# tusen-ai/MV2D

Measured on AMD Instinct MI355X. Metric: multi-view samples/sec (6-cam frames) through the MV2D RoI-head hot path, higher is better.
Workload: dtype f16x3: every operand an fp16 hi + lo pair, three MFMAs per product, fp32 accumulation (fp32-class, index-exact route; the lo halves of the key / value rows are STORED as e4m3 bytes); 1 GPU; cfg2_s: MV2D-S head, 6 views 1408x512; global_batch=384, streams_per_gpu=4, samples_per_launch=16, pe_sine_branch=folded into a per-(weights, geometry) table, FLOPs not counted, parallelism=dp1, hipgraph=True

## Files before the change

include/mv2d_hip.h:

```cpp
#ifndef MV2D_HIP_H
#define MV2D_HIP_H
#ifdef __cplusplus
extern "C" {
#endif

const char* mv2d_last_error(void);
int mv2d_abi_version(void);
int mv2d_key16_format(void);
int mv2d_f32_to_key16(const float* x, void* hi, void* lo, long long n, void* stream);
int mv2d_device_arch(char* buf, int buflen);
int mv2d_spin(int usec, void* stream);


int mv2d_gemm_bf16(const void* A, const void* A2, int n_split, int a_mode, const void* W, const float* bias, int M, int N,
                   int K, int lda, const int* m_dev, int act, const float* mul, int ldmul, const float* add, int ldadd,
                   void* C, int c_bf16, int ldc, long long c_blk_stride, int c_blk_cols, void* C2, const float* add2,
                   int ldc2, int ldadd2, void* stream);
int mv2d_gemm_bf16_ex(const void* A, const void* A2, int n_split, int a_mode, const void* W, const float* bias, int M, int N, int K, int lda,
                      const int* m_dev, int act, const float* mul, int ldmul, const float* add, int ldadd, void* C, int c_bf16, int ldc,
                      long long c_blk_stride, int c_blk_cols, void* C2, const float* add2, int ldc2, int ldadd2, int c_split3, const int* add_idx , int add_period,
                      int k_splits , long long c_split_stride, void* stream);
int mv2d_split3_rows(const float* a, const float* b, void* out, int M, int cols, const int* m_dev, void* stream);

int mv2d_gemm_f32(const float* A, const float* A2, int n_split, const float* W, const float* bias, int M, int N, int K,
// ... 109 lines not shown
int mv2d_split_rows_key16(const float* a, const float* b, void* hi, void* lo, int M, int cols, const int* m_dev, void* stream);

int mv2d_heads_fused_x3(const float* outs, const void* const* cls_w, const void* const* reg_w, const float* ref, float* cls, float* reg,
                        int M, int L, float eps, const float* pc_range, float dt, const float* dt_rows, void* stream);
int mv2d_heads_fused_x3_nc(const float* outs, const void* const* cls_w, const void* const* reg_w, const float* ref, float* cls, float* reg,
                           int M, int L, int num_classes, float eps, const float* pc_range, float dt, const float* dt_rows, void* stream);
int mv2d_heads_cls_x3_nc(const float* outs, const void* const* cls_w, float* cls, int M, int L, int num_classes, float eps, void* stream);
int mv2d_reg_layer_x3(const float* outs, const void* const* w, const float* ref, float* reg, int M, int L, int n_groups, const int* group_dims,
                      const float* pc_range, float dt, const float* dt_rows, void* stream);

int mv2d_heads_depth_x3(const float* outs, const void* const* cls_w, const void* const* reg_w, const float* ref, float* cls, float* reg,
                        int M, int L, int n_fcs, int num_classes, float eps, const float* pc_range, float dt, const float* dt_rows, void* stream);
int mv2d_heads_cls_depth_x3(const float* outs, const void* const* cls_w, float* cls, int M, int L, int n_fcs, int num_classes, float eps,
                            void* stream);
int mv2d_reg_layer_depth_x3(const float* outs, const void* const* w, const float* ref, float* reg, int M, int L, int n_fcs, int n_groups,
                            const int* group_dims, const float* pc_range, float dt, const float* dt_rows, void* stream);

int mv2d_ffn_pack_weights(const float* W1, const float* W2, float* W1p, float* W2p, int hidden, void* stream);
int mv2d_ffn_fused(const float* X, const float* W1, const float* b1, const float* W2, float* slabs, int M, int hidden, void* stream);

int mv2d_ffn_fused_x3(const float* X, const void* W1hi, const void* W1lo, const float* b1, const void* W2hi, const void* W2lo,
                      float* slabs, int M, int hidden, int slices_per_block, void* stream);

int mv2d_split_bf16x2(const float* x, void* hi, void* lo, long long n, void* stream);
int mv2d_q16_format(void);
int mv2d_split_q16x2(const float* x, void* hi, void* lo, long long n, void* stream);


int mv2d_row_ln(const float* parts, int n_parts, long long part_stride, const float* bias, const float* residual,
                const float* ln_w, const float* ln_b, int relu, float* out, const float* addvec, float* out_plus,
                const float* ln2_w, const float* ln2_b, float* out2, int M, float eps, int rows_per_group, void* stream);

int mv2d_finalize_reg(float* reg, const float* ref, int L, int R, const float* pc_range, float dt, void* stream);

int mv2d_avgpool49(const float* x, float* out, int ld_out, int R, void* stream);

int mv2d_f32_to_bf16(const float* x, void* y, long long n, void* stream);

int mv2d_nchw_to_nhwc(const float* x, float* y, int V, int C, int HW, void* stream);
int mv2d_nchw_to_nhwc_masked(const float* x, float* y, const unsigned char* mask, int V, int C, int HW, void* stream);
int mv2d_nchw_to_nhwc_fmt(const void* x, void* y, int V, int C, int HW, int map_fmt, void* stream);
int mv2d_nchw_to_nhwc_masked_fmt(const void* x, void* y, const unsigned char* mask, int V, int C, int HW, int map_fmt, void* stream);

int mv2d_nchw_to_nhwc_bf16(const float* x, void* y, int V, int C, int HW, void* stream);
int mv2d_map_conv3x3(const void* in, const void* Wp, const float* bias, float* out, int V, int h, int w, void* stream);



int mv2d_self_attn_fwd(const float* qkv, float* ctx, int R, const int* grp_start, int n_samples, void* stream);

int mv2d_self_attn_x3_fwd(const float* qkv, float* ctx, int R, const int* grp_start, int n_samples, int max_grp_rows, int dn_pad,
                          int dn_single, void* stream);

int mv2d_self_attn_dn_fwd(const float* qkv, float* ctx, int R, int dn_pad, int dn_single, void* stream);

int mv2d_sparse_xattn_fwd(const float* q, const void* K, const void* V, const int* row_ptr, const int* col_idx, float* ctx,
                          float* dbg_logits, long long dbg_stride, int R, int empty_nan, void* stream);

int mv2d_xattn_qmap(const float* q, const void* WA_hi, const void* WA_lo, void* Qt, int R, void* stream);
int mv2d_xattn_tile_fwd(const void* Qt, const void* Xk, const void* Xv, const void* Xk_lo, const void* Xv_lo, const int* row_ptr,
                        const int* col_idx, float* z, float* dbg_logits, long long dbg_stride, int R, int empty_nan, int waves, void* stream);
int mv2d_xattn_tile_fwd_ordered(const void* Qt, const void* Xk, const void* Xv, const void* Xk_lo, const void* Xv_lo, const int* row_ptr,
                                const int* col_idx, float* z, float* dbg_logits, long long dbg_stride, int R, int empty_nan, int waves,
                                const int* order, int lo_fmt, void* stream);
int mv2d_xattn_fused_fwd(const float* q, const void* WA_hi, const void* WA_lo, const void* WB_hi, const void* WB_lo, const float* bv, const void* Xk,
                         const void* Xv, const void* Xk_lo, const void* Xv_lo, const int* row_ptr, const int* col_idx, float* ctx, int R, int empty_nan,
                         const int* order, int lo_fmt, void* stream);
int mv2d_xattn_group_max(int R, int n_samples);
int mv2d_xattn_group_tables(const int* row_ptr, const int* col_idx, const int* order, const int* grp_start, int n_samples, int R, int ng_max, int* g_slot,
                            int* g_cnt, int* g_ptr, int* g_len, int* ucol, unsigned char* umask, int ucap, int* u_total, int* flags, void* stream);
int mv2d_xattn_group_fwd(const float* q, const void* WA_hi, const void* WA_lo, const void* WB_hi, const void* WB_lo, const float* bv, const void* Xk,
                         const void* Xv, const void* Xk_lo, const void* Xv_lo, const int* row_ptr, const int* order, const int* g_slot, const int* g_cnt,
                         const int* g_ptr, const int* g_len, const int* ucol, const unsigned char* umask, float* ctx, int ng_max, int empty_nan,
                         void* stream);
int mv2d_xattn_ctxmap(const float* z, const void* WB_hi, const void* WB_lo, const float* bv, const int* row_ptr, float* ctx, int R,
                      int empty_nan, void* stream);

int mv2d_xattn_query_order(const int* row_ptr, const int* col_idx, const int* grp_start, int n_samples, int R, int* perm, int* flags, int stride,
                           void* stream);
int mv2d_attn_out_qmap_x3(const float* ctx, const float* resid, const void* Wo_hi, const void* Wo_lo, const float* bo, const float* ln_w,
                          const float* ln_b, float* x_out, const float* qpos, const void* Wq_hi, const void* Wq_lo, const float* bq,
                          float qscale, const void* WA_hi, const void* WA_lo, void* Qt, int M, float eps, void* stream);
int mv2d_attn_out_zmap_x3(const float* z, const void* WB_hi, const void* WB_lo, const float* bv, const int* row_ptr, int empty_nan,
                          const float* resid, const void* Wo_hi, const void* Wo_lo, const float* bo, const float* ln_w, const float* ln_b,
                          float* x_out, int M, float eps, void* stream);

int mv2d_sparse_xattn_bwd(const float* q, const void* K, const void* V, const int* row_ptr, const int* col_idx, const float* ctx,
                          const float* dctx, const int* key_ptr, const int* pair_idx, const int* pair_row, float* pair_ws,
                          float* dq, float* dK, float* dV, int R, int S, void* stream);
int mv2d_sparse_xattn_fwd_drop(const float* q, const void* K, const void* V, const int* row_ptr, const int* col_idx, float* ctx, float* dbg_logits,
                               long long dbg_stride, int R, int empty_nan, float p_drop, unsigned int seed, void* stream);
int mv2d_sparse_xattn_bwd_drop(const float* q, const void* K, const void* V, const int* row_ptr, const int* col_idx, const float* ctx,
                               const float* dctx, const int* key_ptr, const int* pair_idx, const int* pair_row, float* pair_ws, float* dq, float* dK,
                               float* dV, int R, int S, float p_drop, unsigned int seed, void* stream);
int mv2d_sparse_xattn_bwd_ex(const float* q, const void* K, const void* V, const int* row_ptr, const int* col_idx, const float* ctx, const float* dctx,
                             const int* key_ptr, const int* pair_idx, const int* pair_row, float* pair_ws, float* dq, float* dK, float* dV, int R,
                             int S, float p_drop, unsigned int seed, int long_rows, float dq_scale, void* stream);


int mv2d_box_params(const float* rois, const double* viewK, const double* viewE, double* K_roi, float* intr, int ld_intr,
                    float* minv, int R, float roi_size, float intr_scale, float min_size, void* stream);

int mv2d_refpoint_posemb(const float* center_pred, int ld_cp, const float* minv, const float* dim_t, float* xyz, float* ref,
                         float* posemb, int R, const float* pc_range, void* stream);

int mv2d_lidar2img_inverse(const double* K_roi, const double* E, float* minv, int R, void* stream);
// ... 174 lines not shown
```

mv2d_amd/_lib.py:

```python
import ctypes as C
import os

HERE = os.path.dirname(os.path.abspath(__file__))
LIB_PATH = os.path.join(HERE, 'lib', 'libmv2d_hip.so')


class Mv2dHipError(RuntimeError):
    pass


P, I, LL, F, D = C.c_void_p, C.c_int, C.c_longlong, C.c_float, C.c_double
ABI_VERSION = 6

class TdDims(C.Structure):
    _fields_ = [('T', I), ('S', I), ('L', I), ('F', I), ('sa_nnz', I), ('ca_nnz', I), ('p_sa_attn', F), ('p_sa_out', F), ('p_ca_attn', F),
                ('p_ca_out', F), ('p_ffn_act', F), ('p_ffn_out', F), ('seed', C.c_uint), ('eps', F), ('pad', I), ('nk', I)]


class ThDims(C.Structure):
    _fields_ = [('T', I), ('L', I), ('NC', I), ('eps', F)]


SIGNATURES = {
    'mv2d_last_error': (C.c_char_p, []),
# ... 12 lines not shown
    'mv2d_pe_fused_x3_ng': (I, [P, P, P, P, I] + [P] * 7 + [I] + [P] * 5 + [I, I, P, I, I, P]),
    'mv2d_pe_gate_x3': (I, [P, P, P, P, I] + [P] * 7 + [I] + [P] * 5 + [I, I, P]),
    'mv2d_pe_gate_rows_x3': (I, [P, P, P, P, I] + [P] * 7 + [I] + [P] * 5 + [I, P, I, P, I, I, P]),
    'mv2d_pe_fused_x3_k_sel': (I, [P, P, P, P, I] + [P] * 13 + [I] + [P] * 5 + [I, P, I, I, P, I, I, P]),
    'mv2d_pe_fused_x3b': (I, [P, P, P, P, I] + [P] * 13 + [I] + [P] * 5 + [I, I, P, P]),
    'mv2d_key16_format': (I, []),
    'mv2d_f32_to_key16': (I, [P, P, P, LL, P]),
    'mv2d_split_rows_key16': (I, [P, P, P, P, I, I, P, P]),
    'mv2d_qg_conv_pool': (I, [P, P, P, P, I, I, P]),
    'mv2d_qg_conv_pool_x3': (I, [P, P, P, P, P, P, I, I, P]),
    'mv2d_qg_conv_pool_s': (I, [P, P, P, P, I, I, I, P]),
    'mv2d_qg_conv_pool_x3_s': (I, [P, P, P, P, P, P, I, I, I, P]),
    'mv2d_qg_conv_cells': (I, [P, P, P, P, P, P, I, I, P]),
    'mv2d_qg_conv_cells_x3': (I, [P, P, P, P, P, P, P, P, I, I, P]),
    'mv2d_avgpool_cells': (I, [P, P, P, I, I, I, P]),
    'mv2d_pack_wfrag_bf16': (I, [P, P, I, I, P]),
    'mv2d_gemm_f32': (I, [P, P, I, P, P, I, I, I, I, I, I, I, F, F, P, I, I, LL, I, LL, LL, LL, LL, P]),
    'mv2d_attn_out_fused': (I, [P, P, P, P, P, P, P, P, P, P, F, P, I, F, P]),
    'mv2d_sa_block_fused_x3': (I, [P, P, P, P, P, P, P, P, P, P, P, P, F, P, I, F, P]),
    'mv2d_query_embed_fused_x3': (I, [P] * 17 + [I, P]),
    'mv2d_qg_tail_x3': (I, [P, P, I] + [P] * 25 + [I, P]),
    'mv2d_ffn_out_fused_x3': (I, [P, I, LL, P, P, P, P, P, P, P, P, P, P, P, P, P, P, I, F, P]),
    'mv2d_attn_out_fused_x3': (I, [P, P, P, P, P, P, P, P, P, P, P, P, F, P, I, F, P]),
    'mv2d_pack_wfrag_f32': (I, [P, P, I, I, I, P]),
    'mv2d_heads_fused': (I, [P, P, P, P, P, P, I, I, F, P, F, P, P]),
    'mv2d_linear_x3': (I, [P, P, I, I, P, P, P, P, I, I, I, I, I, F, I, LL, LL, LL, LL, P]),
    'mv2d_linear_x3_ex': (I, [P, P, I, I, P, P, P, P, I, I, I, I, I, F, I, LL, LL, LL, LL, P, I, P, P, I, P]),
    'mv2d_heads_fused_x3': (I, [P, P, P, P, P, P, I, I, F, P, F, P, P]),
    'mv2d_heads_fused_x3_nc': (I, [P, P, P, P, P, P, I, I, I, F, P, F, P, P]),
    'mv2d_heads_cls_x3_nc': (I, [P, P, P, I, I, I, F, P]),
    'mv2d_reg_layer_x3': (I, [P, P, P, P, I, I, I, P, P, F, P, P]),
    'mv2d_heads_depth_x3': (I, [P, P, P, P, P, P, I, I, I, I, F, P, F, P, P]),
    'mv2d_heads_cls_depth_x3': (I, [P, P, P, I, I, I, I, F, P]),
    'mv2d_reg_layer_depth_x3': (I, [P, P, P, P, I, I, I, I, P, P, F, P, P]),
    'mv2d_ffn_fused': (I, [P, P, P, P, P, I, I, P]),
    'mv2d_ffn_pack_weights': (I, [P, P, P, P, I, P]),
    'mv2d_ffn_fused_x3': (I, [P, P, P, P, P, P, P, I, I, I, P]),
    'mv2d_split_bf16x2': (I, [P, P, P, LL, P]),
    'mv2d_split_q16x2': (I, [P, P, P, LL, P]),
    'mv2d_q16_format': (I, []),
    'mv2d_row_ln': (I, [P, I, LL, P, P, P, P, I, P, P, P, P, P, P, I, F, I, P]),
    'mv2d_finalize_reg': (I, [P, P, I, I, P, F, P]),
    'mv2d_avgpool49': (I, [P, P, I, I, P]),
    'mv2d_f32_to_bf16': (I, [P, P, LL, P]),
    'mv2d_nchw_to_nhwc': (I, [P, P, I, I, I, P]),
    'mv2d_nchw_to_nhwc_masked': (I, [P, P, P, I, I, I, P]),
    'mv2d_nchw_to_nhwc_fmt': (I, [P, P, I, I, I, I, P]),
    'mv2d_nchw_to_nhwc_masked_fmt': (I, [P, P, P, I, I, I, I, P]),
    'mv2d_nchw_to_nhwc_bf16': (I, [P, P, I, I, I, P]),
    'mv2d_map_conv3x3': (I, [P, P, P, P, I, I, I, P]),
    'mv2d_self_attn_fwd': (I, [P, P, I, P, I, P]),
    'mv2d_self_attn_dn_fwd': (I, [P, P, I, I, I, P]),
    'mv2d_self_attn_x3_fwd': (I, [P, P, I, P, I, I, I, I, P]),
    'mv2d_dn_queries': (I, [P, P, P, I, I, F, F, F, I, P, F, P, P, P, P]),
    'mv2d_sparse_xattn_fwd': (I, [P, P, P, P, P, P, P, LL, I, I, P]),
    'mv2d_sparse_xattn_bwd': (I, [P] * 14 + [I, I, P]),
    'mv2d_sparse_xattn_fwd_drop': (I, [P, P, P, P, P, P, P, LL, I, I, F, C.c_uint, P]),
    'mv2d_sparse_xattn_bwd_drop': (I, [P] * 14 + [I, I, F, C.c_uint, P]),
    'mv2d_sparse_xattn_bwd_ex': (I, [P] * 14 + [I, I, F, C.c_uint, I, F, P]),
    'mv2d_dgrad_relu_f32x3': (I, [P, P, P, F, P, I, I, I, P]),
    'mv2d_xattn_qmap': (I, [P, P, P, P, I, P]),
    'mv2d_attn_out_qmap_x3': (I, [P] * 12 + [F, P, P, P, I, F, P]),
    'mv2d_attn_out_zmap_x3': (I, [P, P, P, P, P, I, P, P, P, P, P, P, P, I, F, P]),
    'mv2d_xattn_tile_fwd': (I, [P, P, P, P, P, P, P, P, P, LL, I, I, I, P]),
    'mv2d_xattn_tile_fwd_ordered': (I, [P, P, P, P, P, P, P, P, P, LL, I, I, I, P, I, P]),
    'mv2d_xattn_fused_fwd': (I, [P, P, P, P, P, P, P, P, P, P, P, P, P, I, I, P, I, P]),
    'mv2d_xattn_group_max': (I, [I, I]),
    'mv2d_xattn_group_tables': (I, [P, P, P, P, I, I, I, P, P, P, P, P, P, I, P, P, P]),
    'mv2d_xattn_group_fwd': (I, [P] * 19 + [I, I, P]),
    'mv2d_xattn_query_order': (I, [P, P, P, I, I, P, P, I, P]),
    'mv2d_xattn_ctxmap': (I, [P, P, P, P, P, P, I, I, P]),
    'mv2d_box_params': (I, [P, P, P, P, P, I, P, I, F, F, F, P]),
    'mv2d_refpoint_posemb': (I, [P, I, P, P, P, P, P, I, P, P]),
    'mv2d_lidar2img_inverse': (I, [P, P, P, I, P]),
    'mv2d_posemb3d': (I, [P, P, P, I, P]),
    'mv2d_roi_align': (I, [P, P, P, P, P, P, P, I, I, I, I, F, I, P, I, P]),
    'mv2d_roi_align_ex': (I, [P, P, P, P, P, P, P, I, I, I, I, F, I, P, I, P, P, P, P, P, P]),
    'mv2d_roi_align_s': (I, [P, P, P, P, P, P, P, I, I, I, I, F, I, P, I, P, P, P, P, P, I, P]),
    'mv2d_roi_align_fmt': (I, [P, P, P, P, P, P, P, I, I, I, I, F, I, P, I, P, P, P, P, P, I, I, P]),
    'mv2d_box_correlation': (I, [P, P, P, P, P, P, I, I, I, I, I, I, I, F, F, F, I, P]),
    'mv2d_csr_workspace_bytes': (LL, [I, I, I, I]),
    'mv2d_mask_compact': (I, [P, P, P, P, P, P, P, P, P, P, P, P, P, I, I, I, I, I, I, F, F, I, P]),
    'mv2d_roi_positions': (I, [P, P, P, P, P, P, P, I, I, I, I, F, F, P]),
    'mv2d_csr_from_corr': (I, [P, P, P, P, I, I, I, P]),
    'mv2d_csr_from_corr_s': (I, [P, P, P, P, I, I, I, I, P]),
    'mv2d_roi_positions_csr': (I, [P, P, P, P, P, P, P, I, I, I, I, F, F, P, P, P, P, I, I, P, I, P, P, P]),
    'mv2d_roi_positions_csr_s': (I, [P, P, P, P, P, P, P, I, I, I, I, F, F, P, P, P, P, I, I, P, I, P, P, I, P]),
    'mv2d_frame_geometry': (I, [P, P, P, P, P, I, P, F, F, F, P, P, P, P, P, I, I, I, I, I, I, I, F, F, F, I, P, LL, P]),
    'mv2d_pe_inputs': (I, [P, P, I, P, P, P, P, P, P, P, P, P, P, P, P, P, I, I, I, I, P, P]),
    'mv2d_pe_inputs_fmt': (I, [P, P, I, P, P, P, P, P, P, P, P, P, P, P, P, P, I, I, I, I, P, I, P]),
    'mv2d_pe_frustum_f32': (I, [P, P, I, P, P, P, P, P, I, I, I, I, P, P]),
    'mv2d_pe_frustum_f32_ld': (I, [P, P, I, P, P, P, P, P, I, I, I, I, P, I, P]),
    'mv2d_pe_frustum_f32_sel': (I, [P, P, I, P, P, P, P, P, I, I, I, I, P, I, P, I, P]),
    'mv2d_pe_inputs_ld': (I, [P, P, I, P, P, P, P, P, P, P, P, P, P, P, P, P, I, I, I, I, P, I, I, P]),
    'mv2d_result_pack': (I, [P, P, P, P, F, I, P, P, P, P, I, I, P]),
    'mv2d_nms_bev': (I, [P, P, P, P, F, P, I, I, P]),
    'mv2d_pack_detections': (I, [P, P, P, P, P, I, I, I, P]),
    'mv2d_roi_align_bwd': (I, [P, P, P, P, I, I, I, I, F, I, P]),
    'mv2d_roi_align_bwd_s': (I, [P, P, P, P, I, I, I, I, F, I, I, P]),
    'mv2d_colsum_scratch_rows': (I, [I]),
    'mv2d_colsum': (I, [P, LL, I, I, P, P, P]),
    'mv2d_gemm_f32x3_ws_bytes': (LL, [I, I, I]),
    'mv2d_gemm_f32x3': (I, [P, LL, I, P, LL, I, P, I, P, LL, I, I, I, P, LL, P]),
    'mv2d_gemm_f32x3_ex': (I, [P, LL, I, P, LL, I, P, I, F, I, I, P, LL, I, I, I, P, LL, P]),
    'mv2d_colsum_add': (I, [P, LL, I, I, P, P, P, P]),
    'mv2d_softmax_bwd_rows': (I, [P, P, P, LL, I, I, F, P]),
# ... 63 lines not shown
```

mv2d_amd/csrc/self_attn_x3.hip:

```cpp
#include "common.h"

namespace {

constexpr int C = 256, HD = 32, KC = 128;
constexpr int VPITCH = KC * 2 + 16;
typedef q16x8_t sa_bf16x8;
union SFrag { uint4 u; sa_bf16x8 v; uint2 h[2]; };

__device__ __forceinline__ void sa_split4(const float4& v, uint2& hi, uint2& lo) {
    split_q16x4(v, hi, lo);
}

template <bool DN>
__global__ __launch_bounds__(256) void self_attn_x3_kernel(const float* __restrict__ qkv, float* __restrict__ ctx, int R, float scale,
                                                           const int* __restrict__ grp_start, int dn_pad, int dn_single, int nx, int npair) {
    __shared__ __attribute__((aligned(16))) unsigned char smem[2 * KC * 64 + 2 * HD * VPITCH];
    unsigned char* Kh = smem;
    unsigned char* Kl = smem + KC * 64;
    unsigned char* Vh = smem + 2 * KC * 64;
    unsigned char* Vl = Vh + HD * VPITCH;
    const int tid = threadIdx.x, lane = tid & 63, wave = tid >> 6, n = lane & 15, g = lane >> 4;
    const int xcd = blockIdx.x & 7, slot = blockIdx.x >> 3, qb = slot % nx, pair = (slot / nx) * 8 + xcd;
    if (pair >= npair) return;
    const int h = pair & 7, grp = pair >> 3;
    if (grp_start) {
        const int gs = grp_start[grp], ge = grp_start[grp + 1];
        qkv += (long long)gs * 768; ctx += (long long)gs * C; R = ge - gs;
    }
    const int q0 = qb * 64 + wave * 16;
    if (qb * 64 >= R) return;
    const bool wave_on = q0 < R;
    SFrag qh, ql;
    {
        const float* qp = qkv + (long long)min(q0 + n, R - 1) * 768 + h * HD + 8 * g;
        float4 a = *reinterpret_cast<const float4*>(qp), b = *reinterpret_cast<const float4*>(qp + 4);
        a = make_float4(a.x * scale, a.y * scale, a.z * scale, a.w * scale);
        b = make_float4(b.x * scale, b.y * scale, b.z * scale, b.w * scale);
        sa_split4(a, qh.h[0], ql.h[0]);
        sa_split4(b, qh.h[1], ql.h[1]);
    }
    float m_run = -INFINITY, l_run = 0.f;
    f32x4_t o0 = {0.f, 0.f, 0.f, 0.f}, o1 = {0.f, 0.f, 0.f, 0.f};
    const int qrow = q0 + n;
    const int qg = (DN && qrow < dn_pad) ? (int)(((float)qrow + 0.5f) / (float)dn_single) : 0;
    const int glo = (DN && qrow < dn_pad) ? qg * dn_single : 0, ghi = (DN && qrow < dn_pad) ? glo + dn_single : 0;
    float4 kreg[KC / 32], vreg[KC / 32];
    auto load_chunk = [&](int k0) {
#pragma unroll
        for (int i = 0; i < KC / 32; ++i) {
            const long long row = (long long)min(k0 + (tid >> 3) + 32 * i, R - 1) * 768 + h * HD + 4 * (tid & 7);
            kreg[i] = *reinterpret_cast<const float4*>(qkv + row + C);
            vreg[i] = *reinterpret_cast<const float4*>(qkv + row + 2 * C);
        }
    };
    load_chunk(0);
    for (int k0 = 0; k0 < R; k0 += KC) {
        if (k0) __syncthreads();
#pragma unroll
        for (int i = 0; i < KC / 32; ++i) {
            const int kr = (tid >> 3) + 32 * i, dq = tid & 7;
            uint2 hi, lo;
            sa_split4(kreg[i], hi, lo);
            const int koff = kr * 64 + ((((dq >> 1) ^ ((kr >> 2) & 3))) << 4) + (dq & 1) * 8;
            *reinterpret_cast<uint2*>(Kh + koff) = hi;
            *reinterpret_cast<uint2*>(Kl + koff) = lo;
            sa_split4(vreg[i], hi, lo);
            const int voff = (4 * dq) * VPITCH + 2 * kr;
            *reinterpret_cast<unsigned short*>(Vh + voff) = (unsigned short)(hi.x & 0xffffu);
            *reinterpret_cast<unsigned short*>(Vh + voff + VPITCH) = (unsigned short)(hi.x >> 16);
            *reinterpret_cast<unsigned short*>(Vh + voff + 2 * VPITCH) = (unsigned short)(hi.y & 0xffffu);
            *reinterpret_cast<unsigned short*>(Vh + voff + 3 * VPITCH) = (unsigned short)(hi.y >> 16);
            *reinterpret_cast<unsigned short*>(Vl + voff) = (unsigned short)(lo.x & 0xffffu);
            *reinterpret_cast<unsigned short*>(Vl + voff + VPITCH) = (unsigned short)(lo.x >> 16);
            *reinterpret_cast<unsigned short*>(Vl + voff + 2 * VPITCH) = (unsigned short)(lo.y & 0xffffu);
            *reinterpret_cast<unsigned short*>(Vl + voff + 3 * VPITCH) = (unsigned short)(lo.y >> 16);
        }
        if (k0 + KC < R) load_chunk(k0 + KC);
        __syncthreads();
        if (!wave_on) continue;
        const int kend = min(KC, R - k0);
        for (int ks = 0; ks < kend; ks += 32) {
            f32x4_t s[2];
#pragma unroll
            for (int t = 0; t < 2; ++t) {
                const int kr = ks + 16 * t + n;
                SFrag kh, kl;
                const int off = kr * 64 + ((g ^ ((kr >> 2) & 3)) << 4);
                kh.u = *reinterpret_cast<const uint4*>(Kh + off);
                kl.u = *reinterpret_cast<const uint4*>(Kl + off);
                f32x4_t a = {0.f, 0.f, 0.f, 0.f};
                a = mfma_q16_16x16x32(kl.v, qh.v, a, 0, 0, 0);
                a = mfma_q16_16x16x32(kh.v, ql.v, a, 0, 0, 0);
                a = mfma_q16_16x16x32(kh.v, qh.v, a, 0, 0, 0);
                s[t] = a;
            }
            float p[8], tmax = -INFINITY;
#pragma unroll
            for (int t = 0; t < 2; ++t)
#pragma unroll
                for (int i = 0; i < 4; ++i) {
                    const int key = k0 + ks + 16 * t + 4 * g + i;
                    bool vis = key < R;
                    if (DN) vis = vis & ((key >= dn_pad) | ((key >= glo) & (key < ghi)));
                    p[4 * t + i] = vis ? s[t][i] : -INFINITY;
                    tmax = fmaxf(tmax, p[4 * t + i]);
                }
            {
                const auto a = __builtin_amdgcn_permlane16_swap(__float_as_uint(tmax), __float_as_uint(tmax), false, false);
                tmax = fmaxf(__uint_as_float(a[0]), __uint_as_float(a[1]));
                const auto b = __builtin_amdgcn_permlane32_swap(__float_as_uint(tmax), __float_as_uint(tmax), false, false);
                tmax = fmaxf(__uint_as_float(b[0]), __uint_as_float(b[1]));
            }
            const float m_new = fmaxf(m_run, tmax);
            const float m_use = (m_new == -INFINITY) ? 0.f : m_new;
            const float alpha = __expf(m_run - m_use);
            float psum = 0.f;
#pragma unroll
            for (int j = 0; j < 8; ++j) { p[j] = __expf(p[j] - m_use); psum += p[j]; }
            {
                const auto a = __builtin_amdgcn_permlane16_swap(__float_as_uint(psum), __float_as_uint(psum), false, false);
                psum = __uint_as_float(a[0]) + __uint_as_float(a[1]);
                const auto b = __builtin_amdgcn_permlane32_swap(__float_as_uint(psum), __float_as_uint(psum), false, false);
                psum = __uint_as_float(b[0]) + __uint_as_float(b[1]);
            }
            l_run = l_run * alpha + psum;
            m_run = m_new;
#pragma unroll
            for (int i = 0; i < 4; ++i) { o0[i] *= alpha; o1[i] *= alpha; }
            SFrag ph, pl;
            sa_split4(make_float4(p[0], p[1], p[2], p[3]), ph.h[0], pl.h[0]);
            sa_split4(make_float4(p[4], p[5], p[6], p[7]), ph.h[1], pl.h[1]);
#pragma unroll
            for (int m = 0; m < 2; ++m) {
                SFrag vh, vl;
                const int off = (16 * m + n) * VPITCH + 2 * (ks + 4 * g);
                vh.h[0] = *reinterpret_cast<const uint2*>(Vh + off);
                vh.h[1] = *reinterpret_cast<const uint2*>(Vh + off + 32);
                vl.h[0] = *reinterpret_cast<const uint2*>(Vl + off);
                vl.h[1] = *reinterpret_cast<const uint2*>(Vl + off + 32);
                f32x4_t& o = m ? o1 : o0;
                o = mfma_q16_16x16x32(vl.v, ph.v, o, 0, 0, 0);
                o = mfma_q16_16x16x32(vh.v, pl.v, o, 0, 0, 0);
                o = mfma_q16_16x16x32(vh.v, ph.v, o, 0, 0, 0);
            }
        }
    }
    if (wave_on && qrow < R) {
        const float inv = 1.0f / l_run;
        float* op = ctx + (long long)qrow * C + h * HD + 4 * g;
        *reinterpret_cast<float4*>(op) = make_float4(o0[0] * inv, o0[1] * inv, o0[2] * inv, o0[3] * inv);
        *reinterpret_cast<float4*>(op + 16) = make_float4(o1[0] * inv, o1[1] * inv, o1[2] * inv, o1[3] * inv);
    }
}

}

extern "C" int mv2d_self_attn_x3_fwd(const float* qkv, float* ctx, int R, const int* grp_start, int n_grp, int max_grp_rows, int dn_pad,
                                     int dn_single, void* stream) {
    MV2D_CHECK_ARG(qkv && ctx && R >= 0 && (!grp_start || n_grp >= 1), "mv2d_self_attn_x3_fwd: bad args");
    MV2D_CHECK_ARG(dn_pad == 0 || (!grp_start && dn_single >= 1 && dn_pad % dn_single == 0 && dn_pad <= R),
                   "mv2d_self_attn_x3_fwd: the denoising mask needs one sample, dn_pad a multiple of dn_single and at most R");
    MV2D_CHECK_ARG(((uintptr_t)qkv & 15) == 0 && ((uintptr_t)ctx & 15) == 0, "mv2d_self_attn_x3_fwd: operands must be 16-byte aligned");
    if (R == 0) return MV2D_OK;
    const int rows = (grp_start && max_grp_rows > 0) ? min(max_grp_rows, R) : R;
    const int nx = cdiv(rows, 64), npair = 8 * (grp_start ? n_grp : 1);
    const dim3 grid(nx * 8 * cdiv(npair, 8));
    const float scale = 1.0f / sqrtf((float)HD);
    if (dn_pad > 0)
        hipLaunchKernelGGL(self_attn_x3_kernel<true>, grid, dim3(256), 0, (hipStream_t)stream, qkv, ctx, R, scale, grp_start, dn_pad, dn_single, nx, npair);
    else
        hipLaunchKernelGGL(self_attn_x3_kernel<false>, grid, dim3(256), 0, (hipStream_t)stream, qkv, ctx, R, scale, grp_start, 0, 1, nx, npair);
    MV2D_LAUNCH_CHECK();
    return MV2D_OK;
}
```

mv2d_amd/ops.py:

```python
import math
import numbers

import torch

from . import _lib
from ._lib import check

BF16 = torch.bfloat16
_K16 = None


def key16_dtype():
    global _K16
    if _K16 is None:
        _K16 = torch.float16 if _lib.load().mv2d_key16_format() == 1 else torch.bfloat16
    return _K16


_RAW_STREAM, _GET_DEV = getattr(torch._C, '_cuda_getCurrentRawStream', None), getattr(torch._C, '_cuda_getDevice', None)


def _stream():
    if _RAW_STREAM is not None and _GET_DEV is not None:
        return _RAW_STREAM(_GET_DEV())
# ... 727 lines not shown
    ld = out.stride(0) if ld_out is None else ld_out
    if out.dtype != torch.float32 or out.numel() < (R - 1) * ld + 256:
        raise ValueError('avgpool_cells: out is an fp32 [R, ld_out >= 256] tensor')
    check(_lib.load().mv2d_avgpool_cells(_p(hi), 0 if lo is None else _p(lo), _p(out), ld, R, cells, _stream()), 'mv2d_avgpool_cells')
    return out


def avgpool49(x, out, ld_out, R):
    check(_lib.load().mv2d_avgpool49(_p(x), _p(out), ld_out, R, _stream()), 'mv2d_avgpool49')
    return out


def f32_to_bf16(x, out=None):
    _req(x, torch.float32, 'x')
    if out is None:
        out = torch.empty(x.shape, device=x.device, dtype=BF16)
    check(_lib.load().mv2d_f32_to_bf16(_p(x), _p(out), x.numel(), _stream()), 'mv2d_f32_to_bf16')
    return out


def nchw_to_nhwc_bf16(x, out=None):
    _req(x, torch.float32, 'x')
    V, Cn, h, w = x.shape
    if out is None:
        out = torch.empty((V * h * w, Cn), device=x.device, dtype=BF16)
    check(_lib.load().mv2d_nchw_to_nhwc_bf16(_p(x), _p(out), V, Cn, h * w, _stream()), 'mv2d_nchw_to_nhwc_bf16')
    return out


def map_conv3x3(x_cl, Wp, bias, V, h, w, out=None):
    _req(x_cl, BF16, 'x_cl'); _req(Wp, BF16, 'Wp'); _req(bias, torch.float32, 'bias')
    if out is None:
        out = torch.empty((V * h * w, 256), device=x_cl.device, dtype=torch.float32)
    check(_lib.load().mv2d_map_conv3x3(_p(x_cl), _p(Wp), _p(bias), _p(out), V, h, w, _stream()), 'mv2d_map_conv3x3')
    return out


def nchw_to_nhwc(x, out=None, mask=None, map_fmt=None):
    fmt = _req_map(x, 'x', map_fmt)
    _req(mask, torch.uint8, 'mask')
    V, Cn, h, w = x.shape
    if out is None:
        if mask is not None:
            raise _lib.Mv2dHipError('nchw_to_nhwc: the masked form writes into a caller-owned buffer')
        out = torch.empty((V * h * w, Cn), device=x.device, dtype=x.dtype)
    _req(out, x.dtype, 'out')
    if mask is not None:
        check(_lib.load().mv2d_nchw_to_nhwc_masked_fmt(_p(x), _p(out), _p(mask), V, Cn, h * w, fmt, _stream()), 'mv2d_nchw_to_nhwc_masked')
    else:
        check(_lib.load().mv2d_nchw_to_nhwc_fmt(_p(x), _p(out), V, Cn, h * w, fmt, _stream()), 'mv2d_nchw_to_nhwc')
    return out


def self_attn(qkv, out=None, R=None, grp_start=None, max_grp_rows=0, impl=None):
    _req(qkv, torch.float32, 'qkv')
    R = qkv.shape[0] if R is None else R
    if out is None:
        out = torch.empty((R, 256), device=qkv.device, dtype=torch.float32)
    n = 0 if grp_start is None else grp_start.numel() - 1
    if (impl or 'x3') == 'x3':
        check(_lib.load().mv2d_self_attn_x3_fwd(_p(qkv), _p(out), R, _p(grp_start), n, int(max_grp_rows), 0, 1, _stream()), 'mv2d_self_attn_x3_fwd')
    else:
        check(_lib.load().mv2d_self_attn_fwd(_p(qkv), _p(out), R, _p(grp_start), n, _stream()), 'mv2d_self_attn_fwd')
    return out


def self_attn_dn(qkv, dn_pad, dn_single, out=None, impl='f32'):
    _req(qkv, torch.float32, 'qkv')
    R = qkv.shape[0]
    if out is None:
        out = torch.empty((R, 256), device=qkv.device, dtype=torch.float32)
    if impl == 'x3':
        check(_lib.load().mv2d_self_attn_x3_fwd(_p(qkv), _p(out), R, None, 0, 0, int(dn_pad), max(int(dn_single), 1), _stream()), 'mv2d_self_attn_x3_fwd')
    else:
        check(_lib.load().mv2d_self_attn_dn_fwd(_p(qkv), _p(out), R, int(dn_pad), int(dn_single), _stream()), 'mv2d_self_attn_dn_fwd')
    return out


def dn_queries(gt, gt_labels, rnd, scalar, noise_scale, noise_trans, split, num_classes, pc_range, eps=1e-4):
    import ctypes
    G = gt.shape[0]
    n = G * scalar
    ref = torch.empty(n, 3, device=gt.device, dtype=torch.float32)
    labels = torch.empty(n, device=gt.device, dtype=torch.int64)
    boxes = torch.empty(n, 9, device=gt.device, dtype=torch.float32)
    rng = (ctypes.c_float * 6)(*[float(x) for x in pc_range])
    check(_lib.load().mv2d_dn_queries(_p(gt), _p(gt_labels), _p(rnd), G, int(scalar), float(noise_scale), float(noise_trans), float(split),
                                      int(num_classes), ctypes.cast(rng, ctypes.c_void_p), float(eps), _p(ref), _p(labels), _p(boxes),
                                      _stream()), 'mv2d_dn_queries')
    return ref, labels, boxes


def sparse_xattn(q, K, V, row_ptr, col_idx, out=None, R=None, dbg_logits=None, empty_nan=True, p_drop=0.0, seed=0):
    _req(q, torch.float32, 'q'); _req(K, BF16, 'K'); _req(V, BF16, 'V')
    _req(row_ptr, torch.int32, 'row_ptr'); _req(col_idx, torch.int32, 'col_idx')
    R = q.shape[0] if R is None else R
    if out is None:
        out = torch.empty((R, 256), device=q.device, dtype=torch.float32)
    check(_lib.load().mv2d_sparse_xattn_fwd_drop(_p(q), _p(K), _p(V), _p(row_ptr), _p(col_idx), _p(out), _p(dbg_logits),
                                                 dbg_logits.stride(0) if dbg_logits is not None else 0, R, 1 if empty_nan else 0, float(p_drop),
                                                 int(seed) & 0xffffffff, _stream()), 'mv2d_sparse_xattn_fwd')
    return out



def pack_xattn_maps(Wk, Wv):
    _req(Wk, torch.float32, 'Wk'); _req(Wv, torch.float32, 'Wv')
    d = Wk.device
    ar = lambda n_: torch.arange(n_, device=d)
    h, t, g, m, e = torch.meshgrid(ar(8), ar(16), ar(4), ar(16), ar(8), indexing='ij')
    wa = Wk[32 * h + 8 * g + e, 32 * (t >> 1) + 8 * (m >> 2) + 4 * (t & 1) + (m & 3)].contiguous()
    h, s, nt, g, n_, e = torch.meshgrid(ar(8), ar(8), ar(2), ar(4), ar(16), ar(8), indexing='ij')
    wb = Wv[32 * h + 16 * nt + n_, 32 * s + 8 * g + e].contiguous()
    return split_q16x2(wa.view(-1)), split_q16x2(wb.view(-1))
# ... 365 lines not shown
```

Measured before the change: 10370 samples/s.

## Add deeper-prefetch self-attention kernel with transposed LDS V reads and wide blocks

New measurement: 10440 samples/s, median of 6. No clear change (+0.6%).

```diff
diff --git a/include/mv2d_hip.h b/include/mv2d_hip.h
--- a/include/mv2d_hip.h
+++ b/include/mv2d_hip.h
@@ -185,6 +185,9 @@
 int mv2d_self_attn_x3_fwd(const float* qkv, float* ctx, int R, const int* grp_start, int n_samples, int max_grp_rows, int dn_pad,
                           int dn_single, void* stream);
 
+int mv2d_self_attn_x3_fwd_form(const float* qkv, float* ctx, int R, const int* grp_start, int n_samples, int max_grp_rows, int dn_pad,
+                               int dn_single, int form, void* stream);
+
 int mv2d_self_attn_dn_fwd(const float* qkv, float* ctx, int R, int dn_pad, int dn_single, void* stream);
 
 int mv2d_sparse_xattn_fwd(const float* q, const void* K, const void* V, const int* row_ptr, const int* col_idx, float* ctx,
diff --git a/mv2d_amd/_lib.py b/mv2d_amd/_lib.py
--- a/mv2d_amd/_lib.py
+++ b/mv2d_amd/_lib.py
@@ -88,6 +88,7 @@
     'mv2d_self_attn_fwd': (I, [P, P, I, P, I, P]),
     'mv2d_self_attn_dn_fwd': (I, [P, P, I, I, I, P]),
     'mv2d_self_attn_x3_fwd': (I, [P, P, I, P, I, I, I, I, P]),
+    'mv2d_self_attn_x3_fwd_form': (I, [P, P, I, P, I, I, I, I, I, P]),
     'mv2d_dn_queries': (I, [P, P, P, I, I, F, F, F, I, P, F, P, P, P, P]),
     'mv2d_sparse_xattn_fwd': (I, [P, P, P, P, P, P, P, LL, I, I, P]),
     'mv2d_sparse_xattn_bwd': (I, [P] * 14 + [I, I, P]),
diff --git a/mv2d_amd/csrc/self_attn_x3.hip b/mv2d_amd/csrc/self_attn_x3.hip
--- a/mv2d_amd/csrc/self_attn_x3.hip
+++ b/mv2d_amd/csrc/self_attn_x3.hip
@@ -1,14 +1,112 @@
 #include "common.h"
 
+#ifdef MV2D_SA_TRACE
+__device__ long long g_sa_trace[32];
+#define SA_STAMP(i) do { if (blockIdx.x == MV2D_SA_TRACE && threadIdx.x == 0) g_sa_trace[i] = (long long)__builtin_amdgcn_s_memtime(); } while (0)
+#define SA_ARRIVED(v) asm volatile("" ::"v"(v))
+__device__ long long g_sa_span[2 * 4096];
+#define SA_SPAN(j) do { if (threadIdx.x == 0 && blockIdx.x < 4096) g_sa_span[2 * blockIdx.x + (j)] = (j) ? (long long)__builtin_amdgcn_s_memrealtime() : sa_t0; } while (0)
+#define SA_SPAN_ENTRY() const long long sa_t0 = (long long)__builtin_amdgcn_s_memrealtime(); if (threadIdx.x == 0 && blockIdx.x < 4096) g_sa_span[2 * blockIdx.x + 1] = 0
+#else
+#define SA_STAMP(i) do {} while (0)
+#define SA_ARRIVED(v) do {} while (0)
+#define SA_SPAN(j) do {} while (0)
+#define SA_SPAN_ENTRY() do {} while (0)
+#endif
+#define SA_CHUNK_STAMP(c, j) SA_STAMP(2 + 4 * min((c), 6) + (j))
+
 namespace {
 
 constexpr int C = 256, HD = 32, KC = 128;
+constexpr int SA_WIDE_BLOCKS = 256;
 constexpr int VPITCH = KC * 2 + 16;
 typedef q16x8_t sa_bf16x8;
+typedef short sa_i16x4 __attribute__((ext_vector_type(4)));
 union SFrag { uint4 u; sa_bf16x8 v; uint2 h[2]; };
 
 __device__ __forceinline__ void sa_split4(const float4& v, uint2& hi, uint2& lo) {
     split_q16x4(v, hi, lo);
+}
+
+__device__ __forceinline__ void sa_load_q(const float* __restrict__ qp, float scale, SFrag& qh, SFrag& ql) {
+    float4 a = *reinterpret_cast<const float4*>(qp), b = *reinterpret_cast<const float4*>(qp + 4);
+    a = make_float4(a.x * scale, a.y * scale, a.z * scale, a.w * scale);
+    b = make_float4(b.x * scale, b.y * scale, b.z * scale, b.w * scale);
+    sa_split4(a, qh.h[0], ql.h[0]);
+    sa_split4(b, qh.h[1], ql.h[1]);
+}
+
+__device__ __forceinline__ int sa_k_off(int kr, int dq) { return kr * 64 + ((((dq >> 1) ^ ((kr >> 2) & 3))) << 4) + (dq & 1) * 8; }
+
+template <bool DN, bool MASK, class VFrag>
+__device__ __forceinline__ void sa_step(const unsigned char* Kh, const unsigned char* Kl, int ks, int key0, int R, int n, int g, const SFrag& qh,
+                                        const SFrag& ql, int dn_pad, int glo, int ghi, float& m_run, float& l_run, f32x4_t& o0, f32x4_t& o1,
+                                        VFrag vfrag) {
+    f32x4_t s[2];
+#pragma unroll
+    for (int t = 0; t < 2; ++t) {
+        const int kr = ks + 16 * t + n;
+        SFrag kh, kl;
+        const int off = kr * 64 + ((g ^ ((kr >> 2) & 3)) << 4);
+        kh.u = *reinterpret_cast<const uint4*>(Kh + off);
+        kl.u = *reinterpret_cast<const uint4*>(Kl + off);
+        f32x4_t a = {0.f, 0.f, 0.f, 0.f};
+        a = mfma_q16_16x16x32(kl.v, qh.v, a, 0, 0, 0);
+        a = mfma_q16_16x16x32(kh.v, ql.v, a, 0, 0, 0);
+        a = mfma_q16_16x16x32(kh.v, qh.v, a, 0, 0, 0);
+        s[t] = a;
+    }
+    float p[8], tmax = -INFINITY;
+#pragma unroll
+    for (int t = 0; t < 2; ++t)
+#pragma unroll
+        for (int i = 0; i < 4; ++i) {
+            const int key = key0 + 16 * t + 4 * g + i;
+            bool vis = !MASK || key < R;
+            if (DN) vis = vis & ((key >= dn_pad) | ((key >= glo) & (key < ghi)));
+            p[4 * t + i] = vis ? s[t][i] : -INFINITY;
+            tmax = fmaxf(tmax, p[4 * t + i]);
+        }
+    {
+        const auto a = __builtin_amdgcn_permlane16_swap(__float_as_uint(tmax), __float_as_uint(tmax), false, false);
+        tmax = fmaxf(__uint_as_float(a[0]), __uint_as_float(a[1]));
+        const auto b = __builtin_amdgcn_permlane32_swap(__float_as_uint(tmax), __float_as_uint(tmax), false, false);
+        tmax = fmaxf(__uint_as_float(b[0]), __uint_as_float(b[1]));
+    }
+    const float m_new = fmaxf(m_run, tmax);
+    const float m_use = (m_new == -INFINITY) ? 0.f : m_new;
+    const float alpha = __expf(m_run - m_use);
+    float psum = 0.f;
+#pragma unroll
+    for (int j = 0; j < 8; ++j) { p[j] = __expf(p[j] - m_use); psum += p[j]; }
+    {
+        const auto a = __builtin_amdgcn_permlane16_swap(__float_as_uint(psum), __float_as_uint(psum), false, false);
+        psum = __uint_as_float(a[0]) + __uint_as_float(a[1]);
+        const auto b = __builtin_amdgcn_permlane32_swap(__float_as_uint(psum), __float_as_uint(psum), false, false);
+        psum = __uint_as_float(b[0]) + __uint_as_float(b[1]);
+    }
+    l_run = l_run * alpha + psum;
+    m_run = m_new;
+#pragma unroll
+    for (int i = 0; i < 4; ++i) { o0[i] *= alpha; o1[i] *= alpha; }
+    SFrag ph, pl;
+    sa_split4(make_float4(p[0], p[1], p[2], p[3]), ph.h[0], pl.h[0]);
+    sa_split4(make_float4(p[4], p[5], p[6], p[7]), ph.h[1], pl.h[1]);
+#pragma unroll
+    for (int m = 0; m < 2; ++m) {
+        SFrag vh, vl;
+        vfrag(m, vh, vl);
+        f32x4_t& o = m ? o1 : o0;
+        o = mfma_q16_16x16x32(vl.v, ph.v, o, 0, 0, 0);
+        o = mfma_q16_16x16x32(vh.v, pl.v, o, 0, 0, 0);
+        o = mfma_q16_16x16x32(vh.v, ph.v, o, 0, 0, 0);
+    }
+}
+
+__device__ __forceinline__ void sa_store(float* __restrict__ op, const f32x4_t& o0, const f32x4_t& o1, float l_run) {
+    const float inv = 1.0f / l_run;
+    *reinterpret_cast<float4*>(op) = make_float4(o0[0] * inv, o0[1] * inv, o0[2] * inv, o0[3] * inv);
+    *reinterpret_cast<float4*>(op + 16) = make_float4(o1[0] * inv, o1[1] * inv, o1[2] * inv, o1[3] * inv);
 }
 
 template <bool DN>
@@ -20,6 +118,8 @@
     unsigned char* Vh = smem + 2 * KC * 64;
     unsigned char* Vl = Vh + HD * VPITCH;
     const int tid = threadIdx.x, lane = tid & 63, wave = tid >> 6, n = lane & 15, g = lane >> 4;
+    SA_SPAN_ENTRY();
+    SA_STAMP(0);
     const int xcd = blockIdx.x & 7, slot = blockIdx.x >> 3, qb = slot % nx, pair = (slot / nx) * 8 + xcd;
     if (pair >= npair) return;
     const int h = pair & 7, grp = pair >> 3;
@@ -31,14 +131,7 @@
     if (qb * 64 >= R) return;
     const bool wave_on = q0 < R;
     SFrag qh, ql;
-    {
-        const float* qp = qkv + (long long)min(q0 + n, R - 1) * 768 + h * HD + 8 * g;
-        float4 a = *reinterpret_cast<const float4*>(qp), b = *reinterpret_cast<const float4*>(qp + 4);
-        a = make_float4(a.x * scale, a.y * scale, a.z * scale, a.w * scale);
-        b = make_float4(b.x * scale, b.y * scale, b.z * scale, b.w * scale);
-        sa_split4(a, qh.h[0], ql.h[0]);
-        sa_split4(b, qh.h[1], ql.h[1]);
-    }
+    sa_load_q(qkv + (long long)min(q0 + n, R - 1) * 768 + h * HD + 8 * g, scale, qh, ql);
     float m_run = -INFINITY, l_run = 0.f;
     f32x4_t o0 = {0.f, 0.f, 0.f, 0.f}, o1 = {0.f, 0.f, 0.f, 0.f};
     const int qrow = q0 + n;
@@ -54,14 +147,17 @@
         }
     };
     load_chunk(0);
+    SA_STAMP(1);
     for (int k0 = 0; k0 < R; k0 += KC) {
         if (k0) __syncthreads();
+        SA_ARRIVED(vreg[KC / 32 - 1].w);
+        SA_CHUNK_STAMP(k0 / KC, 0);
 #pragma unroll
         for (int i = 0; i < KC / 32; ++i) {
             const int kr = (tid >> 3) + 32 * i, dq = tid & 7;
             uint2 hi, lo;
             sa_split4(kreg[i], hi, lo);
-            const int koff = kr * 64 + ((((dq >> 1) ^ ((kr >> 2) & 3))) << 4) + (dq & 1) * 8;
+            const int koff = sa_k_off(kr, dq);
             *reinterpret_cast<uint2*>(Kh + koff) = hi;
             *reinterpret_cast<uint2*>(Kl + koff) = lo;
             sa_split4(vreg[i], hi, lo);
@@ -75,101 +171,179 @@
             *reinterpret_cast<unsigned short*>(Vl + voff + 2 * VPITCH) = (unsigned short)(lo.y & 0xffffu);
             *reinterpret_cast<unsigned short*>(Vl + voff + 3 * VPITCH) = (unsigned short)(lo.y >> 16);
         }
+        SA_CHUNK_STAMP(k0 / KC, 1);
         if (k0 + KC < R) load_chunk(k0 + KC);
         __syncthreads();
+        SA_CHUNK_STAMP(k0 / KC, 2);
         if (!wave_on) continue;
         const int kend = min(KC, R - k0);
-        for (int ks = 0; ks < kend; ks += 32) {
-            f32x4_t s[2];
-#pragma unroll
-            for (int t = 0; t < 2; ++t) {
-                const int kr = ks + 16 * t + n;
-                SFrag kh, kl;
-                const int off = kr * 64 + ((g ^ ((kr >> 2) & 3)) << 4);
-                kh.u = *reinterpret_cast<const uint4*>(Kh + off);
-                kl.u = *reinterpret_cast<const uint4*>(Kl + off);
-                f32x4_t a = {0.f, 0.f, 0.f, 0.f};
-                a = mfma_q16_16x16x32(kl.v, qh.v, a, 0, 0, 0);
-                a = mfma_q16_16x16x32(kh.v, ql.v, a, 0, 0, 0);
-                a = mfma_q16_16x16x32(kh.v, qh.v, a, 0, 0, 0);
-                s[t] = a;
-            }
-            float p[8], tmax = -INFINITY;
-#pragma unroll
-            for (int t = 0; t < 2; ++t)
-#pragma unroll
-                for (int i = 0; i < 4; ++i) {
-                    const int key = k0 + ks + 16 * t + 4 * g + i;
-                    bool vis = key < R;
-                    if (DN) vis = vis & ((key >= dn_pad) | ((key >= glo) & (key < ghi)));
-                    p[4 * t + i] = vis ? s[t][i] : -INFINITY;
-                    tmax = fmaxf(tmax, p[4 * t + i]);
-                }
-            {
-                const auto a = __builtin_amdgcn_permlane16_swap(__float_as_uint(tmax), __float_as_uint(tmax), false, false);
-                tmax = fmaxf(__uint_as_float(a[0]), __uint_as_float(a[1]));
-                const auto b = __builtin_amdgcn_permlane32_swap(__float_as_uint(tmax), __float_as_uint(tmax), false, false);
-                tmax = fmaxf(__uint_as_float(b[0]), __uint_as_float(b[1]));
-            }
-            const float m_new = fmaxf(m_run, tmax);
-            const float m_use = (m_new == -INFINITY) ? 0.f : m_new;
-            const float alpha = __expf(m_run - m_use);
-            float psum = 0.f;
-#pragma unroll
-            for (int j = 0; j < 8; ++j) { p[j] = __expf(p[j] - m_use); psum += p[j]; }
-            {
-                const auto a = __builtin_amdgcn_permlane16_swap(__float_as_uint(psum), __float_as_uint(psum), false, false);
-                psum = __uint_as_float(a[0]) + __uint_as_float(a[1]);
-                const auto b = __builtin_amdgcn_permlane32_swap(__float_as_uint(psum), __float_as_uint(psum), false, false);
-                psum = __uint_as_float(b[0]) + __uint_as_float(b[1]);
-            }
-            l_run = l_run * alpha + psum;
-            m_run = m_new;
-#pragma unroll
-            for (int i = 0; i < 4; ++i) { o0[i] *= alpha; o1[i] *= alpha; }
-            SFrag ph, pl;
-            sa_split4(make_float4(p[0], p[1], p[2], p[3]), ph.h[0], pl.h[0]);
-            sa_split4(make_float4(p[4], p[5], p[6], p[7]), ph.h[1], pl.h[1]);
-#pragma unroll
-            for (int m = 0; m < 2; ++m) {
-                SFrag vh, vl;
+        for (int ks = 0; ks < kend; ks += 32)
+            sa_step<DN, true>(Kh, Kl, ks, k0 + ks, R, n, g, qh, ql, dn_pad, glo, ghi, m_run, l_run, o0, o1, [&](int m, SFrag& vh, SFrag& vl) {
                 const int off = (16 * m + n) * VPITCH + 2 * (ks + 4 * g);
                 vh.h[0] = *reinterpret_cast<const uint2*>(Vh + off);
                 vh.h[1] = *reinterpret_cast<const uint2*>(Vh + off + 32);
                 vl.h[0] = *reinterpret_cast<const uint2*>(Vl + off);
                 vl.h[1] = *reinterpret_cast<const uint2*>(Vl + off + 32);
-                f32x4_t& o = m ? o1 : o0;
-                o = mfma_q16_16x16x32(vl.v, ph.v, o, 0, 0, 0);
-                o = mfma_q16_16x16x32(vh.v, pl.v, o, 0, 0, 0);
-                o = mfma_q16_16x16x32(vh.v, ph.v, o, 0, 0, 0);
+            });
+        SA_CHUNK_STAMP(k0 / KC, 3);
+    }
+    if (wave_on && qrow < R) sa_store(ctx + (long long)qrow * C + h * HD + 4 * g, o0, o1, l_run);
+    SA_STAMP(30);
+    SA_SPAN(0);
+    SA_SPAN(1);
+}
+
+template <int DEPTH, int NW>
+__global__ __launch_bounds__(64 * NW) __attribute__((amdgpu_waves_per_eu((NW == 4 && DEPTH == 3) ? 3 : 4))) void self_attn_x3_kernel_w(const float* __restrict__ qkv, float* __restrict__ ctx, int R, float scale,
+                                                                 const int* __restrict__ grp_start, int nx, int npair) {
+    constexpr int NT = 64 * NW, QB = 16 * NW, RP = NT / 8, NI = KC / RP;
+    static_assert(NI * RP == KC, "a chunk is a whole number of load passes");
+    __shared__ __attribute__((aligned(16))) unsigned char smem[4 * KC * 64];
+    unsigned char* Kh = smem;
+    unsigned char* Kl = smem + KC * 64;
+    unsigned char* Vh = smem + 2 * KC * 64;
+    unsigned char* Vl = smem + 3 * KC * 64;
+    const int tid = threadIdx.x, lane = tid & 63, wave = tid >> 6, n = lane & 15, g = lane >> 4;
+    SA_SPAN_ENTRY();
+    SA_STAMP(0);
+    const int xcd = blockIdx.x & 7, slot = blockIdx.x >> 3, npx = (npair + 7) >> 3, qb = slot / npx, pair = (slot % npx) * 8 + xcd;
+    if (pair >= npair) return;
+    const int h = pair & 7, grp = pair >> 3;
+    if (grp_start) {
+        const int gs = grp_start[grp], ge = grp_start[grp + 1];
+        qkv += (long long)gs * 768; ctx += (long long)gs * C; R = ge - gs;
+    }
+    const int q0 = qb * QB + wave * 16;
+    if (qb * QB >= R) return;
+    const bool wave_on = q0 < R;
+    SFrag qh, ql;
+    sa_load_q(qkv + (long long)min(q0 + n, R - 1) * 768 + h * HD + 8 * g, scale, qh, ql);
+    float m_run = -INFINITY, l_run = 0.f;
+    f32x4_t o0 = {0.f, 0.f, 0.f, 0.f}, o1 = {0.f, 0.f, 0.f, 0.f};
+    const int qrow = q0 + n;
+    const int kr0 = tid >> 3, dq = tid & 7;
+    auto pass_on = [&](int k0, int i) { return RP * i < min(KC, (R - k0 + 31) & ~31); };
+    float4 kreg[DEPTH][NI], vreg[DEPTH][NI];
+    auto load_chunk = [&](float4(&kr)[NI], float4(&vr)[NI], int k0) {
+#pragma unroll
+        for (int i = 0; i < NI; ++i)
+            if (pass_on(k0, i)) {
+                const long long row = (long long)min(k0 + kr0 + RP * i, R - 1) * 768 + h * HD + 4 * dq;
+                kr[i] = *reinterpret_cast<const float4*>(qkv + row + C);
+                vr[i] = *reinterpret_cast<const float4*>(qkv + row + 2 * C);
             }
-        }
-    }
-    if (wave_on && qrow < R) {
-        const float inv = 1.0f / l_run;
-        float* op = ctx + (long long)qrow * C + h * HD + 4 * g;
-        *reinterpret_cast<float4*>(op) = make_float4(o0[0] * inv, o0[1] * inv, o0[2] * inv, o0[3] * inv);
-        *reinterpret_cast<float4*>(op + 16) = make_float4(o1[0] * inv, o1[1] * inv, o1[2] * inv, o1[3] * inv);
-    }
-}
-
-}
-
-extern "C" int mv2d_self_attn_x3_fwd(const float* qkv, float* ctx, int R, const int* grp_start, int n_grp, int max_grp_rows, int dn_pad,
-                                     int dn_single, void* stream) {
+    };
+#pragma unroll
+    for (int d = 0; d < DEPTH; ++d)
+        if (d * KC < R) load_chunk(kreg[d], vreg[d], d * KC);
+    SA_STAMP(1);
+    const int vrd = (4 * g + (n >> 2)) * 64 + 8 * (n & 3);
+    for (int kb = 0; kb < R; kb += DEPTH * KC) {
+#pragma unroll
+        for (int d = 0; d < DEPTH; ++d) {
+            const int k0 = kb + d * KC;
+            if (k0 >= R) break;
+            if (k0) __syncthreads();
+#pragma unroll
+            for (int i = 0; i < NI; ++i)
+                if (pass_on(k0, i)) SA_ARRIVED(vreg[d][i].w);
+            SA_CHUNK_STAMP(k0 / KC, 0);
+#pragma unroll
+            for (int i = 0; i < NI; ++i)
+                if (pass_on(k0, i)) {
+                    const int kr = kr0 + RP * i;
+                    uint2 hi, lo;
+                    sa_split4(kreg[d][i], hi, lo);
+                    const int koff = sa_k_off(kr, dq);
+                    *reinterpret_cast<uint2*>(Kh + koff) = hi;
+                    *reinterpret_cast<uint2*>(Kl + koff) = lo;
+                    sa_split4(vreg[d][i], hi, lo);
+                    const int voff = kr * 64 + ((((dq >> 2) ^ (kr >> 2)) & 1) << 5) + (dq & 3) * 8;
+                    *reinterpret_cast<uint2*>(Vh + voff) = hi;
+                    *reinterpret_cast<uint2*>(Vl + voff) = lo;
+                }
+            SA_CHUNK_STAMP(k0 / KC, 1);
+            if (k0 + DEPTH * KC < R) load_chunk(kreg[d], vreg[d], k0 + DEPTH * KC);
+            __syncthreads();
+            SA_CHUNK_STAMP(k0 / KC, 2);
+            if (wave_on) {
+                const int kend = min(KC, R - k0), kfull = kend & ~31;
+                int ks = 0;
+                auto vfrag = [&](int m, SFrag& vh, SFrag& vl) {
+                    typedef __attribute__((address_space(3))) sa_i16x4* lds_p;
+                    const int off = ks * 64 + vrd + (((m ^ g) & 1) << 5);
+                    vh.h[0] = __builtin_bit_cast(uint2, __builtin_amdgcn_ds_read_tr16_b64_v4i16((lds_p)(Vh + off)));
+                    vh.h[1] = __builtin_bit_cast(uint2, __builtin_amdgcn_ds_read_tr16_b64_v4i16((lds_p)(Vh + off + 16 * 64)));
+                    vl.h[0] = __builtin_bit_cast(uint2, __builtin_amdgcn_ds_read_tr16_b64_v4i16((lds_p)(Vl + off)));
+                    vl.h[1] = __builtin_bit_cast(uint2, __builtin_amdgcn_ds_read_tr16_b64_v4i16((lds_p)(Vl + off + 16 * 64)));
+                };
+                for (; ks < kfull; ks += 32) sa_step<false, false>(Kh, Kl, ks, k0 + ks, R, n, g, qh, ql, 0, 0, 0, m_run, l_run, o0, o1, vfrag);
+                if (ks < kend) sa_step<false, true>(Kh, Kl, ks, k0 + ks, R, n, g, qh, ql, 0, 0, 0, m_run, l_run, o0, o1, vfrag);
+            }
+            SA_CHUNK_STAMP(k0 / KC, 3);
+        }
+    }
+    if (wave_on && qrow < R) sa_store(ctx + (long long)qrow * C + h * HD + 4 * g, o0, o1, l_run);
+    SA_STAMP(30);
+    SA_SPAN(0);
+    SA_SPAN(1);
+}
+
+template <int DEPTH, int NW>
+void sa_launch_w(const float* qkv, float* ctx, int R, float scale, const int* grp_start, int rows, int npair, hipStream_t stream) {
+    const int nx = cdiv(rows, 16 * NW);
+    hipLaunchKernelGGL((self_attn_x3_kernel_w<DEPTH, NW>), dim3(nx * 8 * cdiv(npair, 8)), dim3(64 * NW), 0, stream, qkv, ctx, R, scale, grp_start, nx, npair);
+}
+
+int sa_launch(const float* qkv, float* ctx, int R, const int* grp_start, int n_grp, int max_grp_rows, int dn_pad, int dn_single, int form,
+              void* stream) {
     MV2D_CHECK_ARG(qkv && ctx && R >= 0 && (!grp_start || n_grp >= 1), "mv2d_self_attn_x3_fwd: bad args");
     MV2D_CHECK_ARG(dn_pad == 0 || (!grp_start && dn_single >= 1 && dn_pad % dn_single == 0 && dn_pad <= R),
                    "mv2d_self_attn_x3_fwd: the denoising mask needs one sample, dn_pad a multiple of dn_single and at most R");
     MV2D_CHECK_ARG(((uintptr_t)qkv & 15) == 0 && ((uintptr_t)ctx & 15) == 0, "mv2d_self_attn_x3_fwd: operands must be 16-byte aligned");
+    MV2D_CHECK_ARG(form >= 0 && form <= 3 && (dn_pad == 0 || form <= 1), "mv2d_self_attn_x3_fwd_form: form is 0..3, and 0 or 1 with the denoising mask");
     if (R == 0) return MV2D_OK;
     const int rows = (grp_start && max_grp_rows > 0) ? min(max_grp_rows, R) : R;
-    const int nx = cdiv(rows, 64), npair = 8 * (grp_start ? n_grp : 1);
-    const dim3 grid(nx * 8 * cdiv(npair, 8));
+    const int npair = 8 * (grp_start ? n_grp : 1);
     const float scale = 1.0f / sqrtf((float)HD);
-    if (dn_pad > 0)
-        hipLaunchKernelGGL(self_attn_x3_kernel<true>, grid, dim3(256), 0, (hipStream_t)stream, qkv, ctx, R, scale, grp_start, dn_pad, dn_single, nx, npair);
-    else
-        hipLaunchKernelGGL(self_attn_x3_kernel<false>, grid, dim3(256), 0, (hipStream_t)stream, qkv, ctx, R, scale, grp_start, 0, 1, nx, npair);
+    const hipStream_t st = (hipStream_t)stream;
+    if (dn_pad > 0 || form == 1) {
+        const int nx = cdiv(rows, 64);
+        const dim3 grid(nx * 8 * cdiv(npair, 8));
+        if (dn_pad > 0)
+            hipLaunchKernelGGL(self_attn_x3_kernel<true>, grid, dim3(256), 0, st, qkv, ctx, R, scale, grp_start, dn_pad, dn_single, nx, npair);
+        else
+            hipLaunchKernelGGL(self_attn_x3_kernel<false>, grid, dim3(256), 0, st, qkv, ctx, R, scale, grp_start, 0, 1, nx, npair);
+    } else {
+        const int depth = rows <= KC ? 1 : rows <= 2 * KC ? 2 : 3;
+        const bool wide = form == 3 || (form == 0 && cdiv(rows, 64) * npair >= SA_WIDE_BLOCKS);
+        if (wide) {
+            if (depth == 1) sa_launch_w<1, 8>(qkv, ctx, R, scale, grp_start, rows, npair, st);
+            else if (depth == 2) sa_launch_w<2, 8>(qkv, ctx, R, scale, grp_start, rows, npair, st);
+            else sa_launch_w<3, 8>(qkv, ctx, R, scale, grp_start, rows, npair, st);
+        } else {
+            if (depth == 1) sa_launch_w<1, 4>(qkv, ctx, R, scale, grp_start, rows, npair, st);
+            else if (depth == 2) sa_launch_w<2, 4>(qkv, ctx, R, scale, grp_start, rows, npair, st);
+            else sa_launch_w<3, 4>(qkv, ctx, R, scale, grp_start, rows, npair, st);
+        }
+    }
     MV2D_LAUNCH_CHECK();
     return MV2D_OK;
 }
+
+}
+
+#ifdef MV2D_SA_TRACE
+extern "C" int mv2d_sa_trace_read(long long* host, int n) { return hipMemcpyFromSymbol(host, HIP_SYMBOL(g_sa_trace), n * sizeof(long long)) == hipSuccess ? 0 : -2; }
+extern "C" int mv2d_sa_span_read(long long* host, int n_blocks) { return hipMemcpyFromSymbol(host, HIP_SYMBOL(g_sa_span), 2 * n_blocks * sizeof(long long)) == hipSuccess ? 0 : -2; }
+#endif
+
+extern "C" int mv2d_self_attn_x3_fwd(const float* qkv, float* ctx, int R, const int* grp_start, int n_grp, int max_grp_rows, int dn_pad,
+                                     int dn_single, void* stream) {
+    return sa_launch(qkv, ctx, R, grp_start, n_grp, max_grp_rows, dn_pad, dn_single, 0, stream);
+}
+
+extern "C" int mv2d_self_attn_x3_fwd_form(const float* qkv, float* ctx, int R, const int* grp_start, int n_grp, int max_grp_rows, int dn_pad,
+                                          int dn_single, int form, void* stream) {
+    return sa_launch(qkv, ctx, R, grp_start, n_grp, max_grp_rows, dn_pad, dn_single, form, stream);
+}
diff --git a/mv2d_amd/ops.py b/mv2d_amd/ops.py
--- a/mv2d_amd/ops.py
+++ b/mv2d_amd/ops.py
@@ -803,6 +803,9 @@
     return out
 
 
+SA_X3_FORMS = {'x3_chunked': 1, 'x3_q64': 2, 'x3_q128': 3}
+
+
 def self_attn(qkv, out=None, R=None, grp_start=None, max_grp_rows=0, impl=None):
     _req(qkv, torch.float32, 'qkv')
     R = qkv.shape[0] if R is None else R
@@ -811,6 +814,11 @@
     n = 0 if grp_start is None else grp_start.numel() - 1
     if (impl or 'x3') == 'x3':
         check(_lib.load().mv2d_self_attn_x3_fwd(_p(qkv), _p(out), R, _p(grp_start), n, int(max_grp_rows), 0, 1, _stream()), 'mv2d_self_attn_x3_fwd')
+    elif impl in SA_X3_FORMS:
+        check(_lib.load().mv2d_self_attn_x3_fwd_form(_p(qkv), _p(out), R, _p(grp_start), n, int(max_grp_rows), 0, 1, SA_X3_FORMS[impl], _stream()),
+              'mv2d_self_attn_x3_fwd_form')
+    elif impl != 'f32':
+        raise _lib.Mv2dHipError(f'self_attn: unknown impl {impl!r}')
     else:
         check(_lib.load().mv2d_self_attn_fwd(_p(qkv), _p(out), R, _p(grp_start), n, _stream()), 'mv2d_self_attn_fwd')
     return out
```
